# pvjosue/CWFA

Hardware: AMD Instinct MI355X
Metric: volumes/sec inverse-pass @512×512×96 fp32; NLL match vs ref (1/2/4/8 GPU) (higher is better)
Workload: dtype f32 (storage, accumulation, wavelets, couplings); convolution products on the bf16 matrix cores from an exact three-way bf16 split of both fp32 operands, six products per fp32 product: fp32-equivalent; plain-fp32-MFMA figure: fp32_mfma; 1 GPU; 512x512x96 volume, 4-scale CWFA (CAT blocks, 64 ch) + LRNN inverse, z=0, batch 1/GPU, random-init weights (BASELINE.json configs[2]); precision=split, parallelism=replicated x1 (independent volumes per GPU, no collective)

## Files before the change

cwfa_amd/csrc/conv2d.hip:

```cpp
#include "conv_internal.h"

#include <string.h>
#include <type_traits>

namespace {

template <int KS_, int CK_, int MT_, int NT_, int WM_, int WN_, int XV_ = 1>
struct Cfg {
    static constexpr int KS = KS_, CK = CK_, MT = MT_, NT = NT_, WM = WM_, WN = WN_;
    static constexpr int XV = XV_;
    static_assert(XV_ == 1 || (XV_ == 4 && KS_ == 1), "vector staging needs halo-free tiles");
    static constexpr int PAD = KS / 2;
    static constexpr int NTHREADS = 64 * WM * WN;
    static constexpr int CT = 32 * MT * WM;
    static constexpr int TR = NT * WN;
    static constexpr int TC = 32;
    static constexpr int XR = TR + KS - 1;
    static constexpr int XC = TC + KS - 1;
    static constexpr int XS = CK * XR * XC;
    static constexpr int XS_PAD = (XS + 3) & ~3;
    static constexpr int WS = KS * KS * CK * CT;
    static constexpr int XPT = (XS / XV + NTHREADS - 1) / NTHREADS;
    static constexpr int WPT = (WS / 4 + NTHREADS - 1) / NTHREADS;
    static constexpr int BUF = XS_PAD + WS;
// ... 533 lines not shown
        case EPI_RES_ELU: if constexpr (ALLOWED & (1u << EPI_RES_ELU)) return launch_epi<C, EPI_RES_ELU, PRO>(p, st); break;
        case EPI_PRELU: if constexpr (ALLOWED & (1u << EPI_PRELU)) return launch_epi<C, EPI_PRELU, PRO>(p, st); break;
        case EPI_RES_PRELU: if constexpr (ALLOWED & (1u << EPI_RES_PRELU)) return launch_epi<C, EPI_RES_PRELU, PRO>(p, st); break;
        case EPI_GELU_RES: if constexpr (ALLOWED & (1u << EPI_GELU_RES)) return launch_epi<C, EPI_GELU_RES, PRO>(p, st); break;
        case EPI_UP: if constexpr (ALLOWED & (1u << EPI_UP)) return launch_epi<C, EPI_UP, PRO>(p, st); break;
        case EPI_NONE_BLK8:
            if constexpr (ALLOWED & (1u << EPI_NONE_BLK8)) return launch_epi<C, EPI_NONE_BLK8, PRO>(p, st);
            cwfa_set_error("cwfa_conv2d_f32: out_blocked8 is built for the 1x1 kernels with more than 32 output channels");
            return CWFA_E_SHAPE;
        default: break;
    }
    return launch_epi<C, EPI_GENERIC, PRO>(p, st);
}

template <class C, unsigned ALLOWED, unsigned ALLOWED_PRO>
int launch(const ConvParams& p, int epi, hipStream_t st) {
    if (p.o.in_scale || p.o.in_add) return launch_sel<C, ALLOWED_PRO, true>(p, epi, st);
    return launch_sel<C, ALLOWED, false>(p, epi, st);
}

}
int g_cwfa_split_xcd_map = 1;
int g_cwfa_split_rows16 = 1;
extern int g_cwfa_mip3_ablate;
namespace {

int fill_params(ConvParams& p, const char* name, const float* x, const float* w_packed, float* y, int B, int Cin, int H,
                int W, int Cout, int64_t x_bs, int64_t y_bs, const cwfa_conv_opts* opts) {
    CWFA_REQUIRE(B >= 0 && Cin > 0 && Cout > 0 && H >= 0 && W >= 0, CWFA_E_INVAL, "%s: bad size", name);
    if (B == 0 || H == 0 || W == 0) return 1;
    CWFA_REQUIRE(x && w_packed && y, CWFA_E_INVAL, "%s: null pointer", name);
    CWFA_REQUIRE((int64_t)Cin * H * W < (1ll << 30) && (int64_t)Cout * H * W * (p.o.upshuffle2 ? 1 : 1) < (1ll << 30), CWFA_E_SHAPE, "%s: C*H*W exceeds the 32-bit byte offsets of a tile (2^30 elements per image)", name);
    CWFA_REQUIRE(cwfa_aligned16(w_packed), CWFA_E_ALIGN, "%s: packed weights must be 16-byte aligned", name);
    p.x = x; p.wp = w_packed; p.y = y;
    p.B = B; p.Cin = Cin; p.H = H; p.W = W; p.Cout = Cout;
    p.x_bs = x_bs; p.y_bs = y_bs;
    p.products = g_cwfa_operand == CwfaOperand::split3 ? 6 : 1;
    if (opts) p.o = *opts;
    CWFA_REQUIRE(!(p.o.in_scale && !p.o.in_shift), CWFA_E_INVAL, "%s: in_scale without in_shift", name);
    CWFA_REQUIRE(p.o.act >= 0 && p.o.act <= CWFA_ACT_RELU && p.o.act2 >= 0 && p.o.act2 <= CWFA_ACT_RELU, CWFA_E_INVAL,
                 "%s: bad activation", name);
    CWFA_REQUIRE(!((p.o.act == CWFA_ACT_PRELU || p.o.act2 == CWFA_ACT_PRELU) && !p.o.prelu_alpha), CWFA_E_INVAL,
                 "%s: PReLU without prelu_alpha", name);
    return CWFA_OK;
}

// ... 300 lines not shown
    if (strcmp(name, "winograd_2d") == 0) {
        g_cwfa_wino_2d = value;
        return CWFA_OK;
    }
    if (strcmp(name, "wgrad_split") == 0) {
        g_cwfa_wgrad_split = value != 0;
        return CWFA_OK;
    }
    if (strcmp(name, "wgrad_rows") == 0) {
        g_cwfa_wgrad_rows = value;
        return CWFA_OK;
    }
    if (strcmp(name, "split3x3_xcd_map") == 0) {
        g_cwfa_split_xcd_map = value;
        return CWFA_OK;
    }
    if (strcmp(name, "mip3_ablate") == 0) {
        CWFA_REQUIRE(value >= 0 && value <= 7, CWFA_E_INVAL, "cwfa_set_option: mip3_ablate is a mask of bits 0..2");
        g_cwfa_mip3_ablate = value;
        return CWFA_OK;
    }
    if (strcmp(name, "split3x3_rows16") == 0) {
        g_cwfa_split_rows16 = value;
        return CWFA_OK;
    }
    if (strcmp(name, "split_products") == 0) {
        CWFA_REQUIRE(value == 1 || value == 6, CWFA_E_INVAL, "cwfa_set_option: split_products must be 1 or 6");
        CWFA_REQUIRE(value == 1 || g_cwfa_operand != CwfaOperand::fp16, CWFA_E_INVAL,
                     "cwfa_set_option: split_products = 6 needs split_operand = 0 (the three-piece split is a bf16 format)");
        if (value == 6) g_cwfa_operand = CwfaOperand::split3;
        else if (g_cwfa_operand == CwfaOperand::split3) g_cwfa_operand = CwfaOperand::bf16;
        return CWFA_OK;
    }
    if (strcmp(name, "split_operand") == 0) {
        CWFA_REQUIRE(value == 0 || value == 1, CWFA_E_INVAL, "cwfa_set_option: split_operand must be 0 (bf16) or 1 (fp16)");
        CWFA_REQUIRE(value == 0 || g_cwfa_operand != CwfaOperand::split3, CWFA_E_INVAL,
                     "cwfa_set_option: split_operand = 1 (fp16) needs split_products = 1 (fp16 operands take one product)");
        if (value == 1) g_cwfa_operand = CwfaOperand::fp16;
        else if (g_cwfa_operand == CwfaOperand::fp16) g_cwfa_operand = CwfaOperand::bf16;
        return CWFA_OK;
    }
    cwfa_set_error("cwfa_set_option: unknown option '%s'", name);
    return CWFA_E_INVAL;
}

extern "C" int64_t cwfa_conv2d_packed_floats(int Cout, int Cin, int ks) {
// ... 113 lines not shown
```

cwfa_amd/csrc/conv_split3x3.hip:

```cpp
#include "conv_internal.h"

extern int g_cwfa_split_xcd_map;
extern int g_cwfa_split_rows16;

namespace {

constexpr int TR = 8, TC = 32;

template <int KS, int RPW = 4>
struct XG {
    static constexpr int TRW = 2 * RPW, NT = 2 * RPW;
    static constexpr int PAD = KS / 2, XR = TRW + 2 * PAD, XC = TC + 2 * PAD, NTAP = KS * KS;
    static constexpr int EPK = XR * XC;
    static constexpr int KHB = KS == 7 ? 8512 : RPW == 8 ? 9792 : 5440;
    static constexpr int XPB = 2 * KHB;
    static constexpr int XB = 3 * XPB;
    static constexpr bool SPECIAL = KS == 3 && RPW == 4;
    static constexpr int NEK = SPECIAL ? 2 : 3;
    static_assert(EPK * 16 <= KHB && KHB % 256 == 64 && 2 * EPK <= 512 * NEK, "staging entry map");
    static_assert(!SPECIAL || (EPK > 256 && EPK <= 384), "3x3 staging entry map");
    static_assert(KS == 3 || RPW == 4, "7x7: 8-row tiles");
};

template <int MPW, int KS = 3, int RPW = 4, int WM = 4>
struct Geo {
    static constexpr int CT = 16 * MPW * WM;
    static constexpr int WSL = 3 * 4 * CT * 16;
    static constexpr int LDS = 2 * XG<KS, RPW>::XB + 2 * WSL;
    static_assert(LDS <= 160 * 1024, "LDS budget");
};

struct SParams {
    const float* x;
    const void* wp;
    float* y;
    int B, Cin, H, W, Cout, nchunks, nsteps, tiles_x, ntiles, ctiles, xcd_map;
    int nrun;
    int64_t x_bs, y_bs;
    cwfa_conv_opts o;
    cwfa_couple cp;
};

template <int KS, int RPW>
__host__ __device__ constexpr int tap_off(int buf, int tap) { return buf * XG<KS, RPW>::XB + ((tap / KS) * XG<KS, RPW>::XC + tap % KS) * 16; }

enum { EPI_RUNTIME = -1, EPI_COUPLE = -2 };

template <int MPW, bool SIX, bool ADD, int ACT1, int KS = 3, int RPW = 4, int WM = 4, bool F16 = false>
__global__ __launch_bounds__(512, 1) void conv3x3_split_kernel(SParams p) {
    typedef XG<KS, RPW> G;
    constexpr int XC = G::XC, EPK = G::EPK, KHB = G::KHB, XPB = G::XPB, XB = G::XB, NTAP = G::NTAP, PAD = G::PAD;
    constexpr int WN = 8 / WM, RW = G::TRW / WN, NT = 2 * RW;
    constexpr bool SPECIAL = G::SPECIAL;
    static_assert(SPECIAL || ((MPW == 1 || WM != 4) && !ADD), "7x7 / 16-row tiles: the 64-channel and narrow tilings, without a skip add");
    static_assert(WM == 4 || (((KS == 3 && RPW == 8) || KS == 7) && MPW <= 3 && !ADD && ACT1 != EPI_COUPLE),
                  "narrow tilings: 16-row tile (7x7: 8-row), <= 3 m-tiles per wave");
    static_assert(MPW != 3 || WM != 4, "three m-tiles per wave: the 48- / 96-channel tilings only");
    constexpr int CT = 16 * MPW * WM;
    constexpr int WSL = 3 * 4 * CT * 16;
    extern __shared__ __attribute__((aligned(16))) char lds[];
    const int tid = threadIdx.x, lane = tid & 63, c16 = lane & 15, g = lane >> 4;
    const int wave = __builtin_amdgcn_readfirstlane(tid >> 6);
    const int wm = wave % WM, wn = wave / WM;
    const int HW = p.H * p.W;
    const int plane = HW * 4;
    constexpr unsigned OOB = 0x80000000u;
    constexpr int NQ = SIX ? 3 : 1;
    constexpr int OFF_W = 2 * XB;
    const int b = blockIdx.z;
    int sp, ct;
    if (p.xcd_map && (p.ntiles & 7) == 0) {
        const int xcd = blockIdx.x & 7, slot = blockIdx.x >> 3;
        sp = xcd * (p.ntiles >> 3) + slot / p.ctiles;
        ct = slot % p.ctiles;
    } else {
        sp = blockIdx.x / p.ctiles;
        ct = blockIdx.x % p.ctiles;
    }
    const int row0 = (sp / p.tiles_x) * G::TRW, col0 = (sp % p.tiles_x) * TC;

    constexpr int NEK = G::NEK;
    int ekh[NEK], eidx[NEK];
    bool fin[NEK];
    unsigned fo[NEK];
    if constexpr (SPECIAL) {
        ekh[0] = wave >> 2; eidx[0] = tid & 255; fin[0] = true;
        ekh[1] = (wave >> 1) & 1; eidx[1] = 256 + (tid & 127); fin[1] = wave < 4 && eidx[1] < EPK;
    } else {
#pragma unroll
        for (int k = 0; k < NEK; ++k) {
            const int e = tid + 512 * k;
            ekh[k] = e >= EPK;
            eidx[k] = e - ekh[k] * EPK;
            fin[k] = e < 2 * EPK;
        }
    }
    bool fok[NEK];
#pragma unroll
    for (int k = 0; k < NEK; ++k) {
        const int r = eidx[k] / XC, c = eidx[k] % XC;
        const int gr = row0 + r - PAD, gc = col0 + c - PAD;
// ... 175 lines not shown
                }
            }
        }
        {
            const int nP = P == NTAP - 1 ? 0 : P + 1;
            const int nA = 2 * nP, nB = 2 * nP + 1;
            const int nbufA = nA >= NTAP, ntA = nA - NTAP * nbufA, nbufB = nB >= NTAP, ntB = nB - NTAP * nbufB;
            const int noffA = nbufA * XB + ((ntA / KS) * XC + ntA % KS) * 16, noffB = nbufB * XB + ((ntB / KS) * XC + ntB % KS) * 16;
            read_b(0, blane + (sel ? noffB : noffA), 0);
            CWFA_FENCE();
        }
        asm volatile("s_waitcnt vmcnt(0)" ::: "memory");
        if constexpr (SIX) asm volatile("s_waitcnt lgkmcnt(3)" ::: "memory");
        else asm volatile("s_waitcnt lgkmcnt(1)" ::: "memory");
        __builtin_amdgcn_s_barrier();
        sl ^= 1;
        if (++P == NTAP) {
            P = 0;
            ce += 2;
        }
    }
    asm volatile("s_waitcnt vmcnt(0)" ::: "memory");

    const auto ry = CWFA_RSRC(p.y + (int64_t)b * p.y_bs, p.Cout * plane);
    const auto rr = CWFA_RSRC(p.o.residual ? p.o.residual + (int64_t)b * p.o.res_bs : p.y, p.o.residual ? p.Cout * plane : 0);
    const auto rb = CWFA_RSRC(p.o.bias ? p.o.bias : p.y, p.o.bias ? p.Cout * 4 : 0);
    const bool alpha_pc = p.o.prelu_per_channel != 0;
    const float alpha = (p.o.prelu_alpha && !alpha_pc) ? *p.o.prelu_alpha : 0.f;
    const auto rpa = CWFA_RSRC(alpha_pc ? p.o.prelu_alpha : p.y, alpha_pc ? p.Cout * 4 : 0);
    const int cwave = ct * CT + wm * MPW * 16;
    const unsigned glane = (unsigned)(4 * g) * (unsigned)plane;
    if constexpr (ACT1 == EPI_COUPLE) {
        static_assert(MPW <= 2 && !ADD, "coupling epilogue: narrow tilings only");
        constexpr int NP = MPW == 1 ? 2 : 4;
        const cwfa_couple& cp = p.cp;
        const auto cx = CWFA_RSRC(cp.x + (int64_t)b * cp.x_bs, cp.n * plane);
        const auto cy = CWFA_RSRC(cp.y + (int64_t)b * cp.y_bs, cp.n * plane);
        const unsigned jlane = (unsigned)((MPW == 1 ? 2 : 4) * g) * (unsigned)plane;
        const int jwave = wm * (MPW == 1 ? 8 : 16);
        float bs[NP], bt[NP];
#pragma unroll
        for (int k = 0; k < NP; ++k) {
            const int rs = k, rt = MPW == 1 ? k + 2 : 16 + k;
            bs[k] = __builtin_bit_cast(float, __builtin_amdgcn_raw_buffer_load_b32(rb, (unsigned)(16 * g), (cwave + rs) * 4, 0));
            bt[k] = __builtin_bit_cast(float, __builtin_amdgcn_raw_buffer_load_b32(rb, (unsigned)(16 * g), (cwave + rt) * 4, 0));
        }
        float ssum = 0.f;
#pragma unroll
        for (int nt = 0; nt < NT; ++nt) {
            const int row = row0 + wn * RW + (nt >> 1), col = col0 + 16 * (nt & 1) + c16;
            const bool ok = row < p.H && col < p.W;
            const unsigned po = ok ? (unsigned)((row * p.W + col) * 4) + jlane : OOB;
            float xv[NP];
#pragma unroll
// ... 7 lines not shown
                const float sv = cwfa_soft_clamp(sr * cp.pre_scale, cp.clamp_kind, cp.clamp);
                const float tv = tr * cp.pre_scale;
                const float yv = cp.rev ? (xv[k] - tv) * __expf(-sv) : __expf(sv) * xv[k] + tv;
                __builtin_amdgcn_raw_buffer_store_b32(__builtin_bit_cast(unsigned, yv), cy, po, (jwave + k) * plane, 0);
                ssum += ok ? sv : 0.f;
            }
            CWFA_FENCE();
        }
        if (cp.logdet) {
            const double ws = cwfa_wave_sum((double)ssum);
            double* red = reinterpret_cast<double*>(lds);
            __builtin_amdgcn_s_barrier();
            if (lane == 0) red[wave] = ws;
            __syncthreads();
            if (tid == 0) {
                double tot = 0.0;
#pragma unroll
                for (int w = 0; w < 8; ++w) tot += red[w];
                atomicAdd(&cp.logdet[b], cp.rev ? -tot : tot);
            }
        }
        return;
    }
    const bool outb = p.o.out_blocked8 != 0;
    const bool want_stats = ACT1 != EPI_RUNTIME && p.o.out_stats != nullptr;
    float* red = reinterpret_cast<float*>(lds);
#pragma unroll
    for (int mt = 0; mt < MPW; ++mt) {
        float bias[4];
        float st1[4] = {0.f, 0.f, 0.f, 0.f}, st2[4] = {0.f, 0.f, 0.f, 0.f};
#pragma unroll
        for (int r = 0; r < 4; ++r)
            bias[r] = __builtin_bit_cast(float, __builtin_amdgcn_raw_buffer_load_b32(rb, (unsigned)(16 * g), (cwave + mt * 16 + r) * 4, 0));
        float al[4] = {alpha, alpha, alpha, alpha};
        if (alpha_pc) {
#pragma unroll
            for (int r = 0; r < 4; ++r)
                al[r] = __builtin_bit_cast(float, __builtin_amdgcn_raw_buffer_load_b32(rpa, (unsigned)(16 * g), (cwave + mt * 16 + r) * 4, 0));
        }
        constexpr int RLA = NT < 4 ? NT : 4;
        float rv[ACT1 == EPI_RUNTIME ? NT : 1][4];
        auto load_res = [&](int nt) {
            const int row = row0 + wn * RW + (nt >> 1), col = col0 + 16 * (nt & 1) + c16;
            const unsigned po = (row < p.H && col < p.W) ? (unsigned)((row * p.W + col) * 4) + glane : OOB;
#pragma unroll
            for (int r = 0; r < 4; ++r)
                rv[ACT1 == EPI_RUNTIME ? nt : 0][r] = __builtin_bit_cast(float, __builtin_amdgcn_raw_buffer_load_b32(rr, po, (cwave + mt * 16 + r) * plane, 0));
        };
        if constexpr (ACT1 == EPI_RUNTIME) {
#pragma unroll
            for (int nt = 0; nt < NT; ++nt)
#pragma unroll
                for (int r = 0; r < 4; ++r) rv[nt][r] = 0.f;
            if (p.o.residual) {
#pragma unroll
                for (int nt = 0; nt < RLA; ++nt) load_res(nt);
            }
            CWFA_FENCE();
        }
#pragma unroll
        for (int nt = 0; nt < NT; ++nt) {
            const int row = row0 + wn * RW + (nt >> 1), col = col0 + 16 * (nt & 1) + c16;
            if constexpr (ACT1 == EPI_RUNTIME) {
                if (nt + RLA < NT && p.o.residual) load_res(nt + RLA);
                CWFA_FENCE();
            }
            if constexpr (ACT1 != EPI_RUNTIME) {
                if (outb) {
                    f32x4 o4;
#pragma unroll
                    for (int r = 0; r < 4; ++r) o4[r] = cwfa_act_ct<ACT1>(acc[mt][nt][r] + bias[r], al[r]);
                    const unsigned pb = (row < p.H && col < p.W) ? (unsigned)(((g >> 1) * HW + row * p.W + col) * 32 + (g & 1) * 16) : OOB;
                    cwfa_buffer_store_b128(__builtin_bit_cast(u32x4, o4), ry, pb, (cwave + mt * 16) * plane);
                    continue;
                }
            }
            const unsigned po = (row < p.H && col < p.W) ? (unsigned)((row * p.W + col) * 4) + glane : OOB;
#pragma unroll
            for (int r = 0; r < 4; ++r) {
                const int soff = (cwave + mt * 16 + r) * plane;
                float v = acc[mt][nt][r] + bias[r];
                if constexpr (ACT1 == EPI_RUNTIME) {
                    v = cwfa_act(v, p.o.act, al[r]);
                    v += rv[nt][r];
                    v = cwfa_act(v, p.o.act2, al[r]);
                } else {
                    v = cwfa_act_ct<ACT1>(v, al[r]);
                    if (want_stats) {
                        const float vm = po != OOB ? v : 0.f;
                        st1[r] += vm;
                        st2[r] += vm * vm;
                    }
                }
                __builtin_amdgcn_raw_buffer_store_b32(__builtin_bit_cast(unsigned, v), ry, po, soff, 0);
            }
            CWFA_FENCE();
        }
        if constexpr (ACT1 != EPI_RUNTIME) {
            if (want_stats) {
#pragma unroll
                for (int r = 0; r < 4; ++r) {
                    const float a1 = cwfa_row16_sum(st1[r]), a2 = cwfa_row16_sum(st2[r]);
                    if (c16 == 0) {
                        const int ch = (wm * MPW + mt) * 16 + 4 * g + r;
                        red[(wn * CT + ch) * 2] = a1;
                        red[(wn * CT + ch) * 2 + 1] = a2;
                    }
                }
            }
        }
    }
    if constexpr (ACT1 != EPI_RUNTIME) {
        if (want_stats) {
            asm volatile("s_waitcnt lgkmcnt(0)\n\ts_barrier" ::: "memory");
            const int ch = ct * CT + tid;
            if (tid < CT && ch < p.Cout) {
                double s1 = 0.0, s2 = 0.0;
#pragma unroll
                for (int k = 0; k < WN; ++k) {
                    s1 += (double)red[(k * CT + tid) * 2];
                    s2 += (double)red[(k * CT + tid) * 2 + 1];
                }
                atomicAdd(&p.o.out_stats[2 * ch], s1);
                atomicAdd(&p.o.out_stats[2 * ch + 1], s2);
            }
        }
    }
}

template <int CT, bool F16 = false>
__global__ __launch_bounds__(256) void split3x3_pack_kernel(const float* __restrict__ w, uint4* __restrict__ out, int Cout, int Cin,
                                                            int nchunks, int nsteps, int64_t total, int ntap) {
    const int64_t i = (int64_t)blockIdx.x * blockDim.x + threadIdx.x;
    if (i >= total) return;
    const int col = (int)(i % CT), g = (int)((i / CT) % 4), s = (int)((i / (4 * CT)) % nsteps), ctile = (int)(i / ((int64_t)4 * CT * nsteps));
    const int u = 2 * s + (g >> 1), chunk = u / ntap, tap = u % ntap, co = ctile * CT + col;
    unsigned short pc[3][8];
#pragma unroll
    for (int j = 0; j < 8; ++j) {
        const int ci = chunk * 16 + (g & 1) * 8 + j;
        float v = 0.f;
        if (co < Cout && ci < Cin && chunk < nchunks) v = w[((int64_t)co * Cin + ci) * ntap + tap];
        __bf16 a1, a2, a3;
        if constexpr (F16) {
            cwfa_split3<false, true>(v, a1, a2, a3);
            a2 = a3 = __builtin_bit_cast(__bf16, (unsigned short)0);
        } else {
            cwfa_split3<true>(v, a1, a2, a3);
        }
        pc[0][j] = __builtin_bit_cast(unsigned short, a1);
        pc[1][j] = __builtin_bit_cast(unsigned short, a2);
        pc[2][j] = __builtin_bit_cast(unsigned short, a3);
    }
#pragma unroll
    for (int q = 0; q < 3; ++q) {
        uint4 v4;
        v4.x = pc[q][0] | ((unsigned)pc[q][1] << 16);
        v4.y = pc[q][2] | ((unsigned)pc[q][3] << 16);
        v4.z = pc[q][4] | ((unsigned)pc[q][5] << 16);
        v4.w = pc[q][6] | ((unsigned)pc[q][7] << 16);
        out[(((int64_t)ctile * nsteps + s) * 3 + q) * 4 * CT + g * CT + col] = v4;
    }
}

inline int mpw_of(int Cout) { return Cout > 128 ? 4 : Cout > 96 ? 2 : Cout > 64 ? 3 : Cout > 48 ? 1 : Cout > 32 ? 3 : Cout > 16 ? 2 : 1; }
inline int wm_of(int Cout) { return Cout > 96 ? 4 : Cout > 64 ? 2 : Cout > 48 ? 4 : 1; }
inline int ct_of(int Cout) { return 16 * mpw_of(Cout) * wm_of(Cout); }
inline int nsteps_of(int Cin, int ntap = 9) { return ntap * (((Cin + 15) / 16 + 1) / 2); }

template <int MPW, bool ADD, int ACT1, int KS = 3, int RPW = 4, int WM = 4>
int launch(const SParams& p, hipStream_t stream) {
    typedef Geo<MPW, KS, RPW, WM> G;
    constexpr int TRW = XG<KS, RPW>::TRW;
    const int tiles_y = (p.H + TRW - 1) / TRW, ctiles = (p.Cout + G::CT - 1) / G::CT;
    SParams q = p;
    q.ntiles = p.tiles_x * tiles_y;
    q.ctiles = ctiles;
    q.xcd_map = g_cwfa_split_xcd_map;
    if ((int64_t)q.ntiles * ctiles >= (1ll << 31)) {
        cwfa_set_error("cwfa_conv3x3_split_f32: grid too large");
        return CWFA_E_SHAPE;
    }
    if ((ACT1 == EPI_RUNTIME || ACT1 == EPI_COUPLE) && (p.o.out_stats || p.o.out_blocked8)) {
        cwfa_set_error("cwfa_conv3x3_split_f32: out_stats / out_blocked8 reached a run-time epilogue");
        return CWFA_E_INVAL;
    }
    return cwfa_with_operand([&](auto six, auto f16) -> int {
        constexpr auto kern = &conv3x3_split_kernel<MPW, six, ADD, ACT1, KS, RPW, WM, f16>;
        const int rc = cwfa_max_lds<kern>(G::LDS, "cwfa_conv3x3_split_f32");
        if (rc) return rc;
        hipLaunchKernelGGL(kern, dim3((unsigned)(q.ntiles * ctiles), 1, p.B), dim3(512), G::LDS, stream, q);
// ... 7 lines not shown
    const bool plain = !p.o.residual && p.o.act2 == CWFA_ACT_NONE;
    if (p.o.in_add) {
        if (plain && p.o.act == CWFA_ACT_PRELU) return launch<MPW, true, CWFA_ACT_PRELU>(p, st);
        return launch<MPW, true, EPI_RUNTIME>(p, st);
    }
    if (plain && p.o.act == CWFA_ACT_PRELU) return launch<MPW, false, CWFA_ACT_PRELU>(p, st);
    if (plain && p.o.act == CWFA_ACT_NONE) return launch<MPW, false, CWFA_ACT_NONE>(p, st);
    return launch<MPW, false, EPI_RUNTIME>(p, st);
}

void pack_bank(const float* w, void* packed, int Cout, int Cin, int ct, int ntap, hipStream_t st) {
    const int nchunks = (Cin + 15) / 16, nsteps = nsteps_of(Cin, ntap);
    const int64_t total = (int64_t)((Cout + ct - 1) / ct) * nsteps * 4 * ct;
    cwfa_with_operand([&](auto, auto f16) -> int {
        auto go = [&](auto CT) {
            hipLaunchKernelGGL((split3x3_pack_kernel<decltype(CT)::value, f16>), dim3((unsigned)((total + 255) / 256)), dim3(256), 0, st, w,
                               reinterpret_cast<uint4*>(packed), Cout, Cin, nchunks, nsteps, total, ntap);
        };
        if (ct == 16) go(cwfa_ic<16>{});
        else if (ct == 32) go(cwfa_ic<32>{});
        else if (ct == 48) go(cwfa_ic<48>{});
        else if (ct == 96) go(cwfa_ic<96>{});
        else if (ct == 128) go(cwfa_ic<128>{});
        else if (ct == 256) go(cwfa_ic<256>{});
        else go(cwfa_ic<64>{});
        return CWFA_OK;
    });
}

}

static int couple_row_source(int n, int r) {
    int j, which;
    if (n <= 32) {
        const int wm = r >> 4, g = (r >> 2) & 3, q = r & 3;
        j = 8 * wm + 2 * g + (q & 1);
        which = q >> 1;
    } else {
        const int wm = r >> 5;
        which = (r >> 4) & 1;
        j = 16 * wm + (r & 15);
    }
    return j < n ? which * n + j : -1;
}

extern "C" int cwfa_couple_rows(int n, int* rows) {
    if (n <= 0 || n > 64) return -1;
    const int total = n <= 32 ? 64 : 128;
// ... 21 lines not shown
    CWFA_REQUIRE(!cp->in_blocked8 || (Cin % 8 == 0 && cwfa_aligned16(x) && (x_bs & 3) == 0), CWFA_E_ALIGN,
                 "cwfa_conv3x3_split_couple_f32: blocked input needs Cin %% 8 == 0 and 16-byte alignment");
    p.cp = *cp;
    p.nchunks = (Cin + 15) / 16;
    p.nsteps = nsteps_of(Cin);
    p.nrun = p.nsteps - ((p.nchunks & 1) ? 4 : 0);
    p.tiles_x = (W + TC - 1) / TC;
    CWFA_REQUIRE((int64_t)(Cin + 64) * H * W * 4 < (1ll << 31) && (int64_t)(cp->n + 64) * H * W * 4 < (1ll << 31), CWFA_E_SHAPE,
                 "cwfa_conv3x3_split_couple_f32: one sample's input / active half must stay below 2 GiB");
    CWFA_REQUIRE((int64_t)p.tiles_x * ((H + TR - 1) / TR) < (1ll << 31) && B <= 65535, CWFA_E_SHAPE,
                 "cwfa_conv3x3_split_couple_f32: grid too large");
    hipStream_t st = (hipStream_t)stream;
    if (p.Cout == 64) {
        if (g_cwfa_split_rows16 && H > 8)
            return launch<1, false, EPI_COUPLE, 3, 8>(p, st);
        return launch<1, false, EPI_COUPLE>(p, st);
    }
    return launch<2, false, EPI_COUPLE>(p, st);
}

extern "C" int64_t cwfa_conv3x3_split_packed_bytes(int Cout, int Cin) {
    if (Cout <= 0 || Cin <= 0) return -1;
    const int ct = ct_of(Cout);
    return (int64_t)((Cout + ct - 1) / ct) * nsteps_of(Cin) * 3 * 4 * ct * 16;
}

extern "C" int cwfa_conv3x3_split_pack_f32(const float* w, void* packed, int Cout, int Cin, void* stream) {
    CWFA_REQUIRE(w && packed, CWFA_E_INVAL, "cwfa_conv3x3_split_pack_f32: null pointer");
    CWFA_REQUIRE(Cout > 0 && Cin > 0, CWFA_E_SHAPE, "cwfa_conv3x3_split_pack_f32: bad shape");
    CWFA_REQUIRE(cwfa_aligned16(packed), CWFA_E_ALIGN, "cwfa_conv3x3_split_pack_f32: packed image must be 16-byte aligned");
    pack_bank(w, packed, Cout, Cin, ct_of(Cout), 9, (hipStream_t)stream);
    CWFA_LAUNCH_CHECK("cwfa_conv3x3_split_pack_f32");
    return CWFA_OK;
}

extern "C" int cwfa_conv3x3_split_f32(const float* x, const void* w_packed, float* y, int B, int Cin, int H, int W, int Cout,
                                      int64_t x_bs, int64_t y_bs, const cwfa_conv_opts* opts, void* stream) {
    CWFA_REQUIRE(B >= 0 && Cin > 0 && Cout > 0 && H >= 0 && W >= 0, CWFA_E_INVAL, "cwfa_conv3x3_split_f32: bad size");
    if (B == 0 || H == 0 || W == 0) return CWFA_OK;
    CWFA_REQUIRE(x && w_packed && y, CWFA_E_INVAL, "cwfa_conv3x3_split_f32: null pointer");
    CWFA_REQUIRE(cwfa_aligned16(w_packed), CWFA_E_ALIGN, "cwfa_conv3x3_split_f32: packed weights must be 16-byte aligned");
    SParams p{};
    p.x = x; p.wp = w_packed; p.y = y;
    p.B = B; p.Cin = Cin; p.H = H; p.W = W; p.Cout = Cout; p.x_bs = x_bs; p.y_bs = y_bs;
    if (opts) p.o = *opts;
    CWFA_REQUIRE(!p.o.upshuffle2 && !p.o.in_cat, CWFA_E_SHAPE, "cwfa_conv3x3_split_f32: upshuffle2 / in_cat are 1x1 features");
    CWFA_REQUIRE(!p.o.in_blocked8 || (Cin % 8 == 0 && cwfa_aligned16(x) && (x_bs & 3) == 0 && !p.o.in_add), CWFA_E_ALIGN,
// ... 19 lines not shown
    CWFA_REQUIRE((int64_t)(Cin + 64) * H * W * 4 < (1ll << 31) && (int64_t)(Cout + 64 * mpw) * H * W * 4 < (1ll << 31) &&
                     (int64_t)(p.nsteps + 2) * 3 * 4 * 64 * mpw * 16 < (1ll << 31), CWFA_E_SHAPE,
                 "cwfa_conv3x3_split_f32: one sample's input / output / one cout tile's weights must stay below 2 GiB");
    CWFA_REQUIRE((int64_t)p.tiles_x * ((H + TR - 1) / TR) < (1ll << 31) && B <= 65535, CWFA_E_SHAPE, "cwfa_conv3x3_split_f32: grid too large");
    hipStream_t st = (hipStream_t)stream;
    const int wm = wm_of(Cout);
    if (wm != 4) {
        CWFA_REQUIRE(!p.o.in_scale && !p.o.in_add && !p.o.out_blocked8, CWFA_E_INVAL,
                     "cwfa_conv3x3_split_f32: banks with <= 48 or 65 .. 96 outputs take no load-side prologue and write NCHW");
        const bool plain = !p.o.residual && p.o.act2 == CWFA_ACT_NONE;
        const int epi = plain && p.o.act == CWFA_ACT_NONE ? 0 : plain && p.o.act == CWFA_ACT_PRELU ? 1 : 2;
#define CWFA_NARROW(M, W_)                                                                                                                   \
    do {                                                                                                                                     \
        if (epi == 0) return launch<M, false, CWFA_ACT_NONE, 3, 8, W_>(p, st);                                                               \
        if (epi == 1) return launch<M, false, CWFA_ACT_PRELU, 3, 8, W_>(p, st);                                                              \
        return launch<M, false, EPI_RUNTIME, 3, 8, W_>(p, st);                                                                               \
    } while (0)
        if (mpw == 3 && wm == 2) CWFA_NARROW(3, 2);
        if (mpw == 3) CWFA_NARROW(3, 1);
        if (mpw == 2) CWFA_NARROW(2, 1);
        CWFA_NARROW(1, 1);
#undef CWFA_NARROW
    }
    if (mpw == 4) return launch_epi<4>(p, st);
    if (mpw == 2) return launch_epi<2>(p, st);
    if (g_cwfa_split_rows16 && H > 8 && !p.o.in_scale && !p.o.in_add && !p.o.residual && p.o.act == CWFA_ACT_NONE && p.o.act2 == CWFA_ACT_NONE)
        return launch<2, false, CWFA_ACT_NONE, 3, 8, 2>(p, st);
    if (g_cwfa_split_rows16 && H > 8 && !p.o.in_scale && !p.o.in_add && !p.o.out_stats && !p.o.out_blocked8)
        return launch<2, false, EPI_RUNTIME, 3, 8, 2>(p, st);
    return launch_epi<1>(p, st);
}

extern "C" int64_t cwfa_conv7x7_split_packed_bytes(int Cout, int Cin) {
    if (Cout <= 0 || Cout > 64 || Cin <= 0) return -1;
    return (int64_t)nsteps_of(Cin, 49) * 3 * 4 * 64 * 16;
}

extern "C" int cwfa_conv7x7_split_pack_f32(const float* w, void* packed, int Cout, int Cin, void* stream) {
    CWFA_REQUIRE(w && packed, CWFA_E_INVAL, "cwfa_conv7x7_split_pack_f32: null pointer");
    CWFA_REQUIRE(Cout > 0 && Cout <= 64 && Cin > 0, CWFA_E_SHAPE, "cwfa_conv7x7_split_pack_f32: 1 <= Cout <= 64");
    CWFA_REQUIRE(cwfa_aligned16(packed), CWFA_E_ALIGN, "cwfa_conv7x7_split_pack_f32: packed image must be 16-byte aligned");
    pack_bank(w, packed, Cout, Cin, 64, 49, (hipStream_t)stream);
    CWFA_LAUNCH_CHECK("cwfa_conv7x7_split_pack_f32");
    return CWFA_OK;
}

extern "C" int cwfa_conv7x7_split_f32(const float* x, const void* w_packed, float* y, int B, int Cin, int H, int W, int Cout,
// ... 23 lines not shown
```

Before: 52.16 volumes/s.

## Add flattened-K 3x3 split kernel for small-Cin wide banks and 192-channel tiling

Adds a 3x3 split-bf16 conv kernel that flattens taps and input channels into a single K dimension when 9*Cin is at most 64 and the bank is 256 channels wide. This avoids padding each tap to a 16-channel chunk, which wastes most of the MFMA work when Cin is tiny. Weights are packed a second time in flattened order and appended after the regular packed image, so the packed buffer grows. It also adds a 192-channel tiling (three m-tiles per wave) for banks of 129-192 outputs so they are no longer padded to 256. The epilogue is factored into a shared helper.

```diff
diff --git a/cwfa_amd/csrc/conv2d.hip b/cwfa_amd/csrc/conv2d.hip
--- a/cwfa_amd/csrc/conv2d.hip
+++ b/cwfa_amd/csrc/conv2d.hip
@@ -579,6 +579,8 @@
 }
 int g_cwfa_split_xcd_map = 1;
 int g_cwfa_split_rows16 = 1;
+int g_cwfa_split_flatk = 1;
+int g_cwfa_split_ct192 = 1;
 extern int g_cwfa_mip3_ablate;
 namespace {
 
@@ -925,6 +927,14 @@
     }
     if (strcmp(name, "split3x3_rows16") == 0) {
         g_cwfa_split_rows16 = value;
+        return CWFA_OK;
+    }
+    if (strcmp(name, "split3x3_flatk") == 0) {
+        g_cwfa_split_flatk = value;
+        return CWFA_OK;
+    }
+    if (strcmp(name, "split3x3_ct192") == 0) {
+        g_cwfa_split_ct192 = value;
         return CWFA_OK;
     }
     if (strcmp(name, "split_products") == 0) {
diff --git a/cwfa_amd/csrc/conv_split3x3.hip b/cwfa_amd/csrc/conv_split3x3.hip
--- a/cwfa_amd/csrc/conv_split3x3.hip
+++ b/cwfa_amd/csrc/conv_split3x3.hip
@@ -2,6 +2,8 @@
 
 extern int g_cwfa_split_xcd_map;
 extern int g_cwfa_split_rows16;
+extern int g_cwfa_split_flatk;
+extern int g_cwfa_split_ct192;
 
 namespace {
 
@@ -46,6 +48,139 @@
 
 enum { EPI_RUNTIME = -1, EPI_COUPLE = -2 };
 
+__device__ __forceinline__ void split_block_map(const SParams& p, int& sp, int& ct) {
+    if (p.xcd_map && (p.ntiles & 7) == 0) {
+        const int xcd = blockIdx.x & 7, slot = blockIdx.x >> 3;
+        sp = xcd * (p.ntiles >> 3) + slot / p.ctiles;
+        ct = slot % p.ctiles;
+    } else {
+        sp = blockIdx.x / p.ctiles;
+        ct = blockIdx.x % p.ctiles;
+    }
+}
+
+template <int MPW, int NT, int WM, int ACT1>
+__device__ __forceinline__ void split_epilogue(const SParams& p, const f32x4 (&acc)[MPW][NT], char* lds, int b, int ct, int row0, int col0,
+                                               int wm, int wn) {
+    constexpr int CT = 16 * MPW * WM, WN = 8 / WM, RW = NT / 2;
+    constexpr unsigned OOB = 0x80000000u;
+    const int tid = threadIdx.x, c16 = tid & 15, g = (tid & 63) >> 4;
+    const int HW = p.H * p.W;
+    const int plane = HW * 4;
+    const auto ry = CWFA_RSRC(p.y + (int64_t)b * p.y_bs, p.Cout * plane);
+    const auto rr = CWFA_RSRC(p.o.residual ? p.o.residual + (int64_t)b * p.o.res_bs : p.y, p.o.residual ? p.Cout * plane : 0);
+    const auto rb = CWFA_RSRC(p.o.bias ? p.o.bias : p.y, p.o.bias ? p.Cout * 4 : 0);
+    const bool alpha_pc = p.o.prelu_per_channel != 0;
+    const float alpha = (p.o.prelu_alpha && !alpha_pc) ? *p.o.prelu_alpha : 0.f;
+    const auto rpa = CWFA_RSRC(alpha_pc ? p.o.prelu_alpha : p.y, alpha_pc ? p.Cout * 4 : 0);
+    const int cwave = ct * CT + wm * MPW * 16;
+    const unsigned glane = (unsigned)(4 * g) * (unsigned)plane;
+    const bool outb = p.o.out_blocked8 != 0;
+    const bool want_stats = ACT1 != EPI_RUNTIME && p.o.out_stats != nullptr;
+    float* red = reinterpret_cast<float*>(lds);
+#pragma unroll
+    for (int mt = 0; mt < MPW; ++mt) {
+        float bias[4];
+        float st1[4] = {0.f, 0.f, 0.f, 0.f}, st2[4] = {0.f, 0.f, 0.f, 0.f};
+#pragma unroll
+        for (int r = 0; r < 4; ++r)
+            bias[r] = __builtin_bit_cast(float, __builtin_amdgcn_raw_buffer_load_b32(rb, (unsigned)(16 * g), (cwave + mt * 16 + r) * 4, 0));
+        float al[4] = {alpha, alpha, alpha, alpha};
+        if (alpha_pc) {
+#pragma unroll
+            for (int r = 0; r < 4; ++r)
+                al[r] = __builtin_bit_cast(float, __builtin_amdgcn_raw_buffer_load_b32(rpa, (unsigned)(16 * g), (cwave + mt * 16 + r) * 4, 0));
+        }
+        constexpr int RLA = NT < 4 ? NT : 4;
+        float rv[ACT1 == EPI_RUNTIME ? NT : 1][4];
+        auto load_res = [&](int nt) {
+            const int row = row0 + wn * RW + (nt >> 1), col = col0 + 16 * (nt & 1) + c16;
+            const unsigned po = (row < p.H && col < p.W) ? (unsigned)((row * p.W + col) * 4) + glane : OOB;
+#pragma unroll
+            for (int r = 0; r < 4; ++r)
+                rv[ACT1 == EPI_RUNTIME ? nt : 0][r] = __builtin_bit_cast(float, __builtin_amdgcn_raw_buffer_load_b32(rr, po, (cwave + mt * 16 + r) * plane, 0));
+        };
+        if constexpr (ACT1 == EPI_RUNTIME) {
+#pragma unroll
+            for (int nt = 0; nt < NT; ++nt)
+#pragma unroll
+                for (int r = 0; r < 4; ++r) rv[nt][r] = 0.f;
+            if (p.o.residual) {
+#pragma unroll
+                for (int nt = 0; nt < RLA; ++nt) load_res(nt);
+            }
+            CWFA_FENCE();
+        }
+#pragma unroll
+        for (int nt = 0; nt < NT; ++nt) {
+            const int row = row0 + wn * RW + (nt >> 1), col = col0 + 16 * (nt & 1) + c16;
+            if constexpr (ACT1 == EPI_RUNTIME) {
+                if (nt + RLA < NT && p.o.residual) load_res(nt + RLA);
+                CWFA_FENCE();
+            }
+            if constexpr (ACT1 != EPI_RUNTIME) {
+                if (outb) {
+                    f32x4 o4;
+#pragma unroll
+                    for (int r = 0; r < 4; ++r) o4[r] = cwfa_act_ct<ACT1>(acc[mt][nt][r] + bias[r], al[r]);
+                    const unsigned pb = (row < p.H && col < p.W) ? (unsigned)(((g >> 1) * HW + row * p.W + col) * 32 + (g & 1) * 16) : OOB;
+                    cwfa_buffer_store_b128(__builtin_bit_cast(u32x4, o4), ry, pb, (cwave + mt * 16) * plane);
+                    continue;
+                }
+            }
+            const unsigned po = (row < p.H && col < p.W) ? (unsigned)((row * p.W + col) * 4) + glane : OOB;
+#pragma unroll
+            for (int r = 0; r < 4; ++r) {
+                const int soff = (cwave + mt * 16 + r) * plane;
+                float v = acc[mt][nt][r] + bias[r];
+                if constexpr (ACT1 == EPI_RUNTIME) {
+                    v = cwfa_act(v, p.o.act, al[r]);
+                    v += rv[nt][r];
+                    v = cwfa_act(v, p.o.act2, al[r]);
+                } else {
+                    v = cwfa_act_ct<ACT1>(v, al[r]);
+                    if (want_stats) {
+                        const float vm = po != OOB ? v : 0.f;
+                        st1[r] += vm;
+                        st2[r] += vm * vm;
+                    }
+                }
+                __builtin_amdgcn_raw_buffer_store_b32(__builtin_bit_cast(unsigned, v), ry, po, soff, 0);
+            }
+            CWFA_FENCE();
+        }
+        if constexpr (ACT1 != EPI_RUNTIME) {
+            if (want_stats) {
+#pragma unroll
+                for (int r = 0; r < 4; ++r) {
+                    const float a1 = cwfa_row16_sum(st1[r]), a2 = cwfa_row16_sum(st2[r]);
+                    if (c16 == 0) {
+                        const int ch = (wm * MPW + mt) * 16 + 4 * g + r;
+                        red[(wn * CT + ch) * 2] = a1;
+                        red[(wn * CT + ch) * 2 + 1] = a2;
+                    }
+                }
+            }
+        }
+    }
+    if constexpr (ACT1 != EPI_RUNTIME) {
+        if (want_stats) {
+            asm volatile("s_waitcnt lgkmcnt(0)\n\ts_barrier" ::: "memory");
+            const int ch = ct * CT + tid;
+            if (tid < CT && ch < p.Cout) {
+                double s1 = 0.0, s2 = 0.0;
+#pragma unroll
+                for (int k = 0; k < WN; ++k) {
+                    s1 += (double)red[(k * CT + tid) * 2];
+                    s2 += (double)red[(k * CT + tid) * 2 + 1];
+                }
+                atomicAdd(&p.o.out_stats[2 * ch], s1);
+                atomicAdd(&p.o.out_stats[2 * ch + 1], s2);
+            }
+        }
+    }
+}
+
 template <int MPW, bool SIX, bool ADD, int ACT1, int KS = 3, int RPW = 4, int WM = 4, bool F16 = false>
 __global__ __launch_bounds__(512, 1) void conv3x3_split_kernel(SParams p) {
     typedef XG<KS, RPW> G;
@@ -55,7 +190,7 @@
     static_assert(SPECIAL || ((MPW == 1 || WM != 4) && !ADD), "7x7 / 16-row tiles: the 64-channel and narrow tilings, without a skip add");
     static_assert(WM == 4 || (((KS == 3 && RPW == 8) || KS == 7) && MPW <= 3 && !ADD && ACT1 != EPI_COUPLE),
                   "narrow tilings: 16-row tile (7x7: 8-row), <= 3 m-tiles per wave");
-    static_assert(MPW != 3 || WM != 4, "three m-tiles per wave: the 48- / 96-channel tilings only");
+    static_assert(MPW != 3 || WM != 4 || SPECIAL, "three m-tiles per wave x four channel groups (192 channels): the 8-row 3x3 tile only");
     constexpr int CT = 16 * MPW * WM;
     constexpr int WSL = 3 * 4 * CT * 16;
     extern __shared__ __attribute__((aligned(16))) char lds[];
@@ -69,14 +204,7 @@
     constexpr int OFF_W = 2 * XB;
     const int b = blockIdx.z;
     int sp, ct;
-    if (p.xcd_map && (p.ntiles & 7) == 0) {
-        const int xcd = blockIdx.x & 7, slot = blockIdx.x >> 3;
-        sp = xcd * (p.ntiles >> 3) + slot / p.ctiles;
-        ct = slot % p.ctiles;
-    } else {
-        sp = blockIdx.x / p.ctiles;
-        ct = blockIdx.x % p.ctiles;
-    }
+    split_block_map(p, sp, ct);
     const int row0 = (sp / p.tiles_x) * G::TRW, col0 = (sp % p.tiles_x) * TC;
 
     constexpr int NEK = G::NEK;
@@ -298,14 +426,8 @@
     }
     asm volatile("s_waitcnt vmcnt(0)" ::: "memory");
 
-    const auto ry = CWFA_RSRC(p.y + (int64_t)b * p.y_bs, p.Cout * plane);
-    const auto rr = CWFA_RSRC(p.o.residual ? p.o.residual + (int64_t)b * p.o.res_bs : p.y, p.o.residual ? p.Cout * plane : 0);
     const auto rb = CWFA_RSRC(p.o.bias ? p.o.bias : p.y, p.o.bias ? p.Cout * 4 : 0);
-    const bool alpha_pc = p.o.prelu_per_channel != 0;
-    const float alpha = (p.o.prelu_alpha && !alpha_pc) ? *p.o.prelu_alpha : 0.f;
-    const auto rpa = CWFA_RSRC(alpha_pc ? p.o.prelu_alpha : p.y, alpha_pc ? p.Cout * 4 : 0);
     const int cwave = ct * CT + wm * MPW * 16;
-    const unsigned glane = (unsigned)(4 * g) * (unsigned)plane;
     if constexpr (ACT1 == EPI_COUPLE) {
         static_assert(MPW <= 2 && !ADD, "coupling epilogue: narrow tilings only");
         constexpr int NP = MPW == 1 ? 2 : 4;
@@ -359,113 +481,130 @@
         }
         return;
     }
-    const bool outb = p.o.out_blocked8 != 0;
-    const bool want_stats = ACT1 != EPI_RUNTIME && p.o.out_stats != nullptr;
-    float* red = reinterpret_cast<float*>(lds);
-#pragma unroll
-    for (int mt = 0; mt < MPW; ++mt) {
-        float bias[4];
-        float st1[4] = {0.f, 0.f, 0.f, 0.f}, st2[4] = {0.f, 0.f, 0.f, 0.f};
-#pragma unroll
-        for (int r = 0; r < 4; ++r)
-            bias[r] = __builtin_bit_cast(float, __builtin_amdgcn_raw_buffer_load_b32(rb, (unsigned)(16 * g), (cwave + mt * 16 + r) * 4, 0));
-        float al[4] = {alpha, alpha, alpha, alpha};
-        if (alpha_pc) {
-#pragma unroll
-            for (int r = 0; r < 4; ++r)
-                al[r] = __builtin_bit_cast(float, __builtin_amdgcn_raw_buffer_load_b32(rpa, (unsigned)(16 * g), (cwave + mt * 16 + r) * 4, 0));
-        }
-        constexpr int RLA = NT < 4 ? NT : 4;
-        float rv[ACT1 == EPI_RUNTIME ? NT : 1][4];
-        auto load_res = [&](int nt) {
-            const int row = row0 + wn * RW + (nt >> 1), col = col0 + 16 * (nt & 1) + c16;
-            const unsigned po = (row < p.H && col < p.W) ? (unsigned)((row * p.W + col) * 4) + glane : OOB;
-#pragma unroll
-            for (int r = 0; r < 4; ++r)
-                rv[ACT1 == EPI_RUNTIME ? nt : 0][r] = __builtin_bit_cast(float, __builtin_amdgcn_raw_buffer_load_b32(rr, po, (cwave + mt * 16 + r) * plane, 0));
-        };
-        if constexpr (ACT1 == EPI_RUNTIME) {
-#pragma unroll
-            for (int nt = 0; nt < NT; ++nt)
-#pragma unroll
-                for (int r = 0; r < 4; ++r) rv[nt][r] = 0.f;
-            if (p.o.residual) {
-#pragma unroll
-                for (int nt = 0; nt < RLA; ++nt) load_res(nt);
-            }
-            CWFA_FENCE();
-        }
-#pragma unroll
-        for (int nt = 0; nt < NT; ++nt) {
-            const int row = row0 + wn * RW + (nt >> 1), col = col0 + 16 * (nt & 1) + c16;
-            if constexpr (ACT1 == EPI_RUNTIME) {
-                if (nt + RLA < NT && p.o.residual) load_res(nt + RLA);
-                CWFA_FENCE();
-            }
-            if constexpr (ACT1 != EPI_RUNTIME) {
-                if (outb) {
-                    f32x4 o4;
-#pragma unroll
-                    for (int r = 0; r < 4; ++r) o4[r] = cwfa_act_ct<ACT1>(acc[mt][nt][r] + bias[r], al[r]);
-                    const unsigned pb = (row < p.H && col < p.W) ? (unsigned)(((g >> 1) * HW + row * p.W + col) * 32 + (g & 1) * 16) : OOB;
-                    cwfa_buffer_store_b128(__builtin_bit_cast(u32x4, o4), ry, pb, (cwave + mt * 16) * plane);
-                    continue;
+    split_epilogue<MPW, NT, WM, ACT1>(p, acc, lds, b, ct, row0, col0, wm, wn);
+}
+
+struct FlatGeo {
+    static constexpr int CT = 256, WSL = 3 * 4 * CT * 16;
+    static constexpr int KGB = 256 * 16 + 64;
+    static constexpr int BPB = 4 * KGB, BB = 3 * BPB;
+    static constexpr int LDS = BB + 2 * WSL;
+    static_assert(LDS <= 160 * 1024, "LDS budget");
+};
+
+template <bool SIX, int ACT1, bool F16 = false>
+__global__ __launch_bounds__(512, 1) void conv3x3_flatk_kernel(SParams p) {
+    static_assert(ACT1 == CWFA_ACT_NONE || ACT1 == CWFA_ACT_PRELU, "flattened-K form: compile-time bias / PReLU epilogues only");
+    typedef FlatGeo G;
+    constexpr int MPW = 4, WM = 4, RW = 4, NT = 8, CT = G::CT, WSL = G::WSL, KGB = G::KGB, BPB = G::BPB, OFF_W = G::BB;
+    constexpr int NQ = SIX ? 3 : 1;
+    constexpr unsigned OOB = 0x80000000u;
+    extern __shared__ __attribute__((aligned(16))) char lds[];
+    const int tid = threadIdx.x, lane = tid & 63, c16 = lane & 15, g = lane >> 4;
+    const int wave = __builtin_amdgcn_readfirstlane(tid >> 6);
+    const int wm = wave % WM, wn = wave / WM;
+    const int plane = p.H * p.W * 4;
+    const int b = blockIdx.z;
+    int sp, ct;
+    split_block_map(p, sp, ct);
+    const int row0 = (sp / p.tiles_x) * TR, col0 = (sp % p.tiles_x) * TC;
+    const int nst = p.nsteps, K = 9 * p.Cin;
+
+    const int px = tid & 255, pr = row0 + (px >> 5), pcol = col0 + (px & 31), kh = wave >> 2;
+    const auto rx = CWFA_RSRC(p.x + (int64_t)b * p.x_bs, p.Cin * plane);
+    float xv[2][2][8];
+#pragma unroll
+    for (int s = 0; s < 2; ++s)
+#pragma unroll
+        for (int e = 0; e < 2; ++e) {
+            const int k0 = s * 32 + (2 * kh + e) * 8;
+            int tap = k0 / p.Cin, ch = k0 - tap * p.Cin;
+#pragma unroll
+            for (int j = 0; j < 8; ++j) {
+                const int gr = pr + tap / 3 - 1, gc = pcol + tap % 3 - 1;
+                const bool ok = k0 + j < K && s < nst && gr >= 0 && gr < p.H && gc >= 0 && gc < p.W;
+                xv[s][e][j] = __builtin_bit_cast(float, __builtin_amdgcn_raw_buffer_load_b32(rx, ok ? (unsigned)((gr * p.W + gc) * 4) : OOB, ch * plane, 0));
+                if (++ch == p.Cin) {
+                    ch = 0;
+                    ++tap;
                 }
             }
-            const unsigned po = (row < p.H && col < p.W) ? (unsigned)((row * p.W + col) * 4) + glane : OOB;
-#pragma unroll
-            for (int r = 0; r < 4; ++r) {
-                const int soff = (cwave + mt * 16 + r) * plane;
-                float v = acc[mt][nt][r] + bias[r];
-                if constexpr (ACT1 == EPI_RUNTIME) {
-                    v = cwfa_act(v, p.o.act, al[r]);
-                    v += rv[nt][r];
-                    v = cwfa_act(v, p.o.act2, al[r]);
-                } else {
-                    v = cwfa_act_ct<ACT1>(v, al[r]);
-                    if (want_stats) {
-                        const float vm = po != OOB ? v : 0.f;
-                        st1[r] += vm;
-                        st2[r] += vm * vm;
+        }
+    constexpr int NPC = (SIX ? WSL : WSL / 3) / 1024;
+    const auto rw = CWFA_RSRC(reinterpret_cast<const char*>(p.wp) + (int64_t)ct * nst * WSL, nst * WSL);
+    for (int s = 0; s < nst; ++s)
+        cwfa_static_for<NPC / 8>([&](auto ic_) {
+            const int piece = decltype(ic_)::value * 8 + wave;
+            __builtin_amdgcn_raw_ptr_buffer_load_lds(rw, (lds_ptr)(lds + OFF_W + s * WSL + piece * 1024), 16, (unsigned)(lane * 16), s * WSL + piece * 1024, 0, 0);
+        });
+    static_assert(NPC % 8 == 0, "weight slice pieces per wave");
+    auto store_b = [&](const float (&v)[2][8]) {
+#pragma unroll
+        for (int e = 0; e < 2; ++e) {
+            bf16x8 pc[3];
+#pragma unroll
+            for (int j = 0; j < 8; ++j) {
+                __bf16 a1, a2 = (__bf16)0.f, a3 = (__bf16)0.f;
+                cwfa_split3<SIX, F16>(v[e][j], a1, a2, a3);
+                pc[0][j] = a1; pc[1][j] = a2; pc[2][j] = a3;
+            }
+            char* dst = lds + (2 * kh + e) * KGB + px * 16;
+#pragma unroll
+            for (int q = 0; q < NQ; ++q) *reinterpret_cast<bf16x8*>(dst + q * BPB) = pc[q];
+        }
+    };
+
+    f32x4 acc[MPW][NT];
+#pragma unroll
+    for (int mt = 0; mt < MPW; ++mt)
+#pragma unroll
+        for (int nt = 0; nt < NT; ++nt) acc[mt][nt] = f32x4{0.f, 0.f, 0.f, 0.f};
+    const int alane = OFF_W + (g * CT + wm * MPW * 16 + c16) * 16;
+    const int blane = g * KGB + (wn * RW * TC + c16) * 16;
+    auto step = [&](int s) {
+#pragma unroll
+        for (int m0 = 0; m0 < MPW; m0 += 2) {
+            bf16x8 A[2][3], Bq[3];
+#pragma unroll
+            for (int mt = 0; mt < 2; ++mt)
+#pragma unroll
+                for (int q = 0; q < NQ; ++q) A[mt][q] = *reinterpret_cast<const bf16x8*>(lds + alane + s * WSL + (q * 4 * CT + (m0 + mt) * 16) * 16);
+#pragma unroll
+            for (int nt = 0; nt < NT; ++nt) {
+#pragma unroll
+                for (int q = 0; q < NQ; ++q) Bq[q] = *reinterpret_cast<const bf16x8*>(lds + blane + q * BPB + ((nt >> 1) * TC + 16 * (nt & 1)) * 16);
+#pragma unroll
+                for (int mt = 0; mt < 2; ++mt) {
+                    f32x4& c = acc[m0 + mt][nt];
+                    if constexpr (SIX) {
+                        CWFA_MFMA(A[mt][2], Bq[0], c);
+                        CWFA_MFMA(A[mt][1], Bq[1], c);
+                        CWFA_MFMA(A[mt][0], Bq[2], c);
+                        CWFA_MFMA(A[mt][1], Bq[0], c);
+                        CWFA_MFMA(A[mt][0], Bq[1], c);
                     }
+                    CWFA_MFMA_OP(F16, A[mt][0], Bq[0], c);
                 }
-                __builtin_amdgcn_raw_buffer_store_b32(__builtin_bit_cast(unsigned, v), ry, po, soff, 0);
-            }
-            CWFA_FENCE();
-        }
-        if constexpr (ACT1 != EPI_RUNTIME) {
-            if (want_stats) {
-#pragma unroll
-                for (int r = 0; r < 4; ++r) {
-                    const float a1 = cwfa_row16_sum(st1[r]), a2 = cwfa_row16_sum(st2[r]);
-                    if (c16 == 0) {
-                        const int ch = (wm * MPW + mt) * 16 + 4 * g + r;
-                        red[(wn * CT + ch) * 2] = a1;
-                        red[(wn * CT + ch) * 2 + 1] = a2;
-                    }
-                }
-            }
-        }
-    }
-    if constexpr (ACT1 != EPI_RUNTIME) {
-        if (want_stats) {
-            asm volatile("s_waitcnt lgkmcnt(0)\n\ts_barrier" ::: "memory");
-            const int ch = ct * CT + tid;
-            if (tid < CT && ch < p.Cout) {
-                double s1 = 0.0, s2 = 0.0;
-#pragma unroll
-                for (int k = 0; k < WN; ++k) {
-                    s1 += (double)red[(k * CT + tid) * 2];
-                    s2 += (double)red[(k * CT + tid) * 2 + 1];
-                }
-                atomicAdd(&p.o.out_stats[2 * ch], s1);
-                atomicAdd(&p.o.out_stats[2 * ch + 1], s2);
-            }
-        }
-    }
-}
-
-template <int CT, bool F16 = false>
+            }
+        }
+    };
+
+    store_b(xv[0]);
+    asm volatile("s_waitcnt vmcnt(0)\n\ts_waitcnt lgkmcnt(0)" ::: "memory");
+    __builtin_amdgcn_s_barrier();
+    step(0);
+    if (nst > 1) {
+        __builtin_amdgcn_s_barrier();
+        store_b(xv[1]);
+        asm volatile("s_waitcnt lgkmcnt(0)" ::: "memory");
+        __builtin_amdgcn_s_barrier();
+        step(1);
+    }
+    __builtin_amdgcn_s_barrier();
+    split_epilogue<MPW, NT, WM, ACT1>(p, acc, lds, b, ct, row0, col0, wm, wn);
+}
+
+template <int CT, bool F16 = false, bool FLAT = false>
 __global__ __launch_bounds__(256) void split3x3_pack_kernel(const float* __restrict__ w, uint4* __restrict__ out, int Cout, int Cin,
                                                             int nchunks, int nsteps, int64_t total, int ntap) {
     const int64_t i = (int64_t)blockIdx.x * blockDim.x + threadIdx.x;
@@ -475,9 +614,14 @@
     unsigned short pc[3][8];
 #pragma unroll
     for (int j = 0; j < 8; ++j) {
-        const int ci = chunk * 16 + (g & 1) * 8 + j;
         float v = 0.f;
-        if (co < Cout && ci < Cin && chunk < nchunks) v = w[((int64_t)co * Cin + ci) * ntap + tap];
+        if constexpr (FLAT) {
+            const int k = 32 * s + 8 * g + j;
+            if (co < Cout && k < ntap * Cin) v = w[((int64_t)co * Cin + k % Cin) * ntap + k / Cin];
+        } else {
+            const int ci = chunk * 16 + (g & 1) * 8 + j;
+            if (co < Cout && ci < Cin && chunk < nchunks) v = w[((int64_t)co * Cin + ci) * ntap + tap];
+        }
         __bf16 a1, a2, a3;
         if constexpr (F16) {
             cwfa_split3<false, true>(v, a1, a2, a3);
@@ -500,10 +644,16 @@
     }
 }
 
-inline int mpw_of(int Cout) { return Cout > 128 ? 4 : Cout > 96 ? 2 : Cout > 64 ? 3 : Cout > 48 ? 1 : Cout > 32 ? 3 : Cout > 16 ? 2 : 1; }
+inline int mpw_of(int Cout) {
+    if (Cout > 128 && Cout <= 192 && g_cwfa_split_ct192) return 3;
+    return Cout > 128 ? 4 : Cout > 96 ? 2 : Cout > 64 ? 3 : Cout > 48 ? 1 : Cout > 32 ? 3 : Cout > 16 ? 2 : 1;
+}
 inline int wm_of(int Cout) { return Cout > 96 ? 4 : Cout > 64 ? 2 : Cout > 48 ? 4 : 1; }
 inline int ct_of(int Cout) { return 16 * mpw_of(Cout) * wm_of(Cout); }
 inline int nsteps_of(int Cin, int ntap = 9) { return ntap * (((Cin + 15) / 16 + 1) / 2); }
+inline bool flatk_bank(int Cout, int Cin) { return 9 * Cin <= 64 && ct_of(Cout) == FlatGeo::CT; }
+inline int flatk_steps(int Cin) { return 9 * Cin <= 32 ? 1 : 2; }
+inline int64_t regular_bytes(int Cout, int Cin) { const int ct = ct_of(Cout); return (int64_t)((Cout + ct - 1) / ct) * nsteps_of(Cin) * 3 * 4 * ct * 16; }
 
 template <int MPW, bool ADD, int ACT1, int KS = 3, int RPW = 4, int WM = 4>
 int launch(const SParams& p, hipStream_t stream) {
@@ -557,8 +707,39 @@
         else if (ct == 48) go(cwfa_ic<48>{});
         else if (ct == 96) go(cwfa_ic<96>{});
         else if (ct == 128) go(cwfa_ic<128>{});
+        else if (ct == 192) go(cwfa_ic<192>{});
         else if (ct == 256) go(cwfa_ic<256>{});
         else go(cwfa_ic<64>{});
+        if (ntap == 9 && flatk_bank(Cout, Cin)) {
+            const int fst = flatk_steps(Cin);
+            const int64_t ftotal = (int64_t)((Cout + ct - 1) / ct) * fst * 4 * ct;
+            hipLaunchKernelGGL((split3x3_pack_kernel<FlatGeo::CT, f16, true>), dim3((unsigned)((ftotal + 255) / 256)), dim3(256), 0, st, w,
+                               reinterpret_cast<uint4*>(reinterpret_cast<char*>(packed) + regular_bytes(Cout, Cin)), Cout, Cin, nchunks, fst,
+                               ftotal, ntap);
+        }
+        return CWFA_OK;
+    });
+}
+
+template <int ACT1>
+int launch_flat(const SParams& p, hipStream_t stream) {
+    typedef FlatGeo G;
+    SParams q = p;
+    q.ctiles = (p.Cout + G::CT - 1) / G::CT;
+    q.ntiles = p.tiles_x * ((p.H + TR - 1) / TR);
+    q.xcd_map = g_cwfa_split_xcd_map;
+    q.wp = reinterpret_cast<const char*>(p.wp) + regular_bytes(p.Cout, p.Cin);
+    q.nsteps = q.nrun = flatk_steps(p.Cin);
+    if ((int64_t)q.ntiles * q.ctiles >= (1ll << 31)) {
+        cwfa_set_error("cwfa_conv3x3_split_f32: grid too large");
+        return CWFA_E_SHAPE;
+    }
+    return cwfa_with_operand([&](auto six, auto f16) -> int {
+        constexpr auto kern = &conv3x3_flatk_kernel<six, ACT1, f16>;
+        const int rc = cwfa_max_lds<kern>(G::LDS, "cwfa_conv3x3_split_f32");
+        if (rc) return rc;
+        hipLaunchKernelGGL(kern, dim3((unsigned)(q.ntiles * q.ctiles), 1, p.B), dim3(512), G::LDS, stream, q);
+        CWFA_LAUNCH_CHECK("cwfa_conv3x3_split_f32");
         return CWFA_OK;
     });
 }
@@ -626,7 +807,7 @@
 extern "C" int64_t cwfa_conv3x3_split_packed_bytes(int Cout, int Cin) {
     if (Cout <= 0 || Cin <= 0) return -1;
     const int ct = ct_of(Cout);
-    return (int64_t)((Cout + ct - 1) / ct) * nsteps_of(Cin) * 3 * 4 * ct * 16;
+    return regular_bytes(Cout, Cin) + (flatk_bank(Cout, Cin) ? (int64_t)((Cout + ct - 1) / ct) * flatk_steps(Cin) * FlatGeo::WSL : 0);
 }
 
 extern "C" int cwfa_conv3x3_split_pack_f32(const float* w, void* packed, int Cout, int Cin, void* stream) {
@@ -692,7 +873,14 @@
         CWFA_NARROW(1, 1);
 #undef CWFA_NARROW
     }
+    if (g_cwfa_split_flatk && flatk_bank(Cout, Cin) && !p.o.in_scale && !p.o.in_add && !p.o.in_blocked8 && !p.o.residual &&
+        p.o.act2 == CWFA_ACT_NONE && (p.o.act == CWFA_ACT_NONE || p.o.act == CWFA_ACT_PRELU)) {
+        CWFA_REQUIRE(!(p.o.out_stats || p.o.out_blocked8) || p.o.act == CWFA_ACT_NONE || p.o.act == CWFA_ACT_PRELU, CWFA_E_INVAL,
+                     "cwfa_conv3x3_split_f32: out_stats / out_blocked8 reached the flattened-K form without a compile-time epilogue");
+        return p.o.act == CWFA_ACT_PRELU ? launch_flat<CWFA_ACT_PRELU>(p, st) : launch_flat<CWFA_ACT_NONE>(p, st);
+    }
     if (mpw == 4) return launch_epi<4>(p, st);
+    if (mpw == 3) return launch_epi<3>(p, st);
     if (mpw == 2) return launch_epi<2>(p, st);
     if (g_cwfa_split_rows16 && H > 8 && !p.o.in_scale && !p.o.in_add && !p.o.residual && p.o.act == CWFA_ACT_NONE && p.o.act2 == CWFA_ACT_NONE)
         return launch<2, false, CWFA_ACT_NONE, 3, 8, 2>(p, st);
```

Result: no change. 52.33 volumes/s (median of 6 runs) (+0.3%).
